# smellslikeml/distributed-deep-learning-workshop

Hardware: AMD Instinct MI355X
Metric: images/sec (whole node) ResNet-50 224px (higher is better)
Workload: dtype bf16; 1 GPU; model=resnet50, global_batch=256, per_gpu_batch=256, image_size=224, parallelism=dp1, hip_ops=True, conv_routes=hip

## Files before the change

ddlw_amd/ops/abi.py:

```python
from __future__ import annotations

import ctypes
from ctypes import POINTER, c_char_p, c_float, c_int, c_long, c_ulonglong


class Ptr(ctypes.c_void_p):

    @classmethod
    def from_param(cls, v):
        if v is None or isinstance(v, int):
            return ctypes.c_void_p(v)
        return ctypes.c_void_p(v.data_ptr())


def long_array(values):
    return (c_long * len(values))(*values)


def int_array(values):
    return (c_int * len(values))(*values)


_P, _I, _L, _F = Ptr, c_int, c_long, c_float

# ... 9 lines not shown
    "ddlw_bn_grad_finalize": (_I, [_P, _P, _P, _P, _I, _I, _P]),
    "ddlw_bn_bwd_dx": (_I, [_P] * 10 + [_L, _I, _I, _P]),
    "ddlw_maxpool3x3s2_fwd": (_I, [_P, _P, _P] + [_I] * 6 + [_P]),
    "ddlw_maxpool3x3s2_bwd": (_I, [_P, _P, _P] + [_I] * 6 + [_P]),
    "ddlw_gap_fwd": (_I, [_P, _P, _I, _I, _I, _P]),
    "ddlw_gap_bwd": (_I, [_P, _P, _I, _I, _I, _P]),
    "ddlw_softmax_ce": (_I, [_P, _P, _P, _P, _I, _I, _F, _P]),
    "ddlw_dropout_fwd": (_I, [_P, _P, _P, _L, _F, c_ulonglong, _P]),
    "ddlw_dropout_bwd": (_I, [_P, _P, _P, _L, _F, _P]),
    "ddlw_argmax_rows": (_I, [_P, _P, _L, _I, _P]),
    "ddlw_accuracy": (_I, [_P, _P, _P, _L, _I, _P]),
    "ddlw_normalize_u8": (_I, [_P, _P, _L, _P]),
    "ddlw_fused_sgd": (_I, [_P, _I, _L, _F, _F, _F, _I, _P]),
    "ddlw_fused_adam": (_I, [_P, _I, _L, _F, _F, _F, _F, _F, _F, _F, _P]),
    "ddlw_depthwise_fwd": (_I, [_P, _P, _P] + [_I] * 10 + [_P]),
    "ddlw_depthwise_fwd_ep": (_I, [_P] * 5 + [_I] * 9 + [_P]),
    "ddlw_depthwise_dgrad": (_I, [_P, _P, _P] + [_I] * 10 + [_P]),
    "ddlw_depthwise_wgrad_nparts": (_I, [_L, _I]),
    "ddlw_depthwise_wgrad": (_I, [_P, _P, _P, _P] + [_I] * 10 + [_P]),
    "ddlw_pw_conv_fwd": (_I, [_P] * 6 + [_I, _L, _I, _I, _P]),
    "ddlw_pw_conv_nparts": (_I, [_L, _I, _P]),
    "ddlw_pw_conv_fwd_stats": (_I, [_P] * 5 + [_L, _I, _I, _P]),
    "ddlw_conv_fwd_nparts": (_L, [_I] * 8),
    "ddlw_conv_fwd_igemm": (_I, [_P] * 13 + [_I] * 15 + [_P]),
    "ddlw_conv_dgrad_s2m": (_I, [_P] * 4 + [_I] * 9
                            + [POINTER(c_long), POINTER(c_long), POINTER(c_int), _P]),
    "ddlw_conv_wgrad": (_I, [_P] * 5 + [_I] * 12 + [_P]),
    "ddlw_stem_repack": (_I, [_P, _P, _I, _I, _I, _P]),
    "ddlw_conv_stem": (_I, [_P] * 4 + [_I] * 8 + [_P, _P, _I, _P]),
    "ddlw_stem_wgrad": (_I, [_P] * 5 + [_I] * 7 + [_P]),
}


def apply(cdll, on_missing) -> None:
    for name, (restype, argtypes) in SIGNATURES.items():
        try:
            fn = getattr(cdll, name)
        except AttributeError:
            on_missing(name)
            raise
        fn.restype = restype
        fn.argtypes = argtypes
```

ddlw_amd/ops/block.py:

```python
from __future__ import annotations

import os

import torch

from . import binding, conv_gemm


def fused_block_enabled() -> bool:
    return os.environ.get("DDLW_FUSED_BLOCK", "1") == "1"


def wgrad_stream_enabled() -> bool:
    return os.environ.get("DDLW_WGRAD_STREAM", "0") == "1"


_wgrad_streams = {}


def _wgrad_stream(device) -> "torch.cuda.Stream":
    s = _wgrad_streams.get(device)
    if s is None:
        s = _wgrad_streams[device] = torch.cuda.Stream(device=device)
    return s


def _cl(t: torch.Tensor) -> torch.Tensor:
    return t.contiguous(memory_format=torch.channels_last)


def _fwd_conv(x, w, stride, padding, hip_fwd):
    if hip_fwd:
        return conv_gemm.conv_fwd_kernel(x, w.to(torch.bfloat16), stride, padding)
    return torch.nn.functional.conv2d(x, w.to(x.dtype), None, stride, padding)


def _dgrad_bn_reduce(dy, conv_in, weight, stride, padding, hip_dgrad,
                     x_bn, mask, mean, rstd):
    st = stride[0] if isinstance(stride, (tuple, list)) else stride
    if (hip_dgrad and st == 1
            and os.environ.get("DDLW_FUSED_BNB", "1") == "1"):
        dx, parts, np_ = conv_gemm.conv_dgrad_kernel(
            dy, weight.to(torch.bfloat16), conv_in.shape, padding, stride,
            bnb=(x_bn, mask, mean, rstd))
        db, dg = binding.bn_grad_finalize_parts(
            parts[0], parts[1], np_, x_bn.shape[1])
        return dx, db, dg
# ... 2 lines not shown
    db, dg = binding.bn_bwd_reduce(dx, mask, x_bn, mean, rstd,
                                   mask is not None)
    return dx, db, dg


def _fwd_conv_bn_stats(x, w, stride, padding, hip_fwd, bn):
    if hip_fwd and os.environ.get("DDLW_FUSED_BN_STATS", "1") == "1":
        t, parts, np_ = conv_gemm.conv_fwd_kernel(
            x, w.to(torch.bfloat16), stride, padding, bn_parts=True)
        rows = t.shape[0] * t.shape[2] * t.shape[3]
        mean, rstd = binding.bn_finalize_parts(
            parts[0], parts[1], np_, rows, t.shape[1], bn.eps, bn.momentum,
            bn.running_mean, bn.running_var)
        return t, mean, rstd
    t = _fwd_conv(x, w, stride, padding, hip_fwd)
    mean, rstd = binding.bn_stats(t, bn.eps, bn.momentum,
                                  bn.running_mean, bn.running_var)
    return t, mean, rstd


class _BottleneckFn(torch.autograd.Function):

    @staticmethod
    def forward(ctx, x, w1, g1, b1, w2, g2, b2, w3, g3, b3, wd, gd, bd, block):
        bn1, bn2, bn3 = block.bn1, block.bn2, block.bn3
        stride = block.stride
        mode = os.environ.get("DDLW_CONV", "auto")
        x = _cl(x)

        if wd is not None:
            dsc = block.downsample.conv
            dsbn = block.downsample.bn
            conv_gemm.available(dsc, x, mode)
            rdf, rdd, rdg = getattr(dsc, "_ddlw_route", (False, False, False))
            td, md, sd = _fwd_conv_bn_stats(x, wd, stride, 0, rdf, dsbn)
            res, _ = binding.bn_apply(td, None, md, sd, gd, bd, False)
            dsbn.num_batches_tracked += 1
        else:
            rdd = rdg = False
            td = md = sd = None
            res = x

        conv_gemm.available(block.conv1, x, mode)
        r1f, r1d, r1g = getattr(block.conv1, "_ddlw_route", (False, False, False))
        t1, m1, s1 = _fwd_conv_bn_stats(x, w1, 1, 0, r1f, bn1)
        a1, mask1 = binding.bn_apply(t1, None, m1, s1, g1, b1, True)

        conv_gemm.available(block.conv2, a1, mode)
        r2f, r2d, r2g = getattr(block.conv2, "_ddlw_route", (False, False, False))
        t2, m2, s2 = _fwd_conv_bn_stats(a1, w2, stride, 1, r2f, bn2)
        a2, mask2 = binding.bn_apply(t2, None, m2, s2, g2, b2, True)

        conv_gemm.available(block.conv3, a2, mode)
        r3f, r3d, r3g = getattr(block.conv3, "_ddlw_route", (False, False, False))
        t3, m3, s3 = _fwd_conv_bn_stats(a2, w3, 1, 0, r3f, bn3)
        out, mask3 = binding.bn_apply(t3, res, m3, s3, g3, b3, True)

        for bn in (bn1, bn2, bn3):
            bn.num_batches_tracked += 1
        ctx.save_for_backward(x, w1, g1, w2, g2, w3, g3, wd, gd,
                              t1, a1, t2, a2, t3, td,
                              mask1, mask2, mask3,
                              m1, s1, m2, s2, m3, s3, md, sd)
        ctx.routes = ((r1d, r1g), (r2d, r2g), (r3d, r3g), (rdd, rdg))
        ctx.stride = stride
        return out

    @staticmethod
    def backward(ctx, dy):
        (x, w1, g1, w2, g2, w3, g3, wd, gd,
         t1, a1, t2, a2, t3, td,
         mask1, mask2, mask3,
         m1, s1, m2, s2, m3, s3, md, sd) = ctx.saved_tensors
        (r1d, r1g), (r2d, r2g), (r3d, r3g), (rdd, rdg) = ctx.routes
        stride = ctx.stride
        dy = _cl(dy)
        if dy.dtype != torch.bfloat16:
            dy = dy.to(torch.bfloat16)

        use_side = wgrad_stream_enabled() and dy.is_cuda
        main = torch.cuda.current_stream() if use_side else None
        side = _wgrad_stream(dy.device) if use_side else None
        side_evs = []

        def wgrad(dy_t, x_t, w, st, pd, hip_g):
            if not use_side:
                _, dw = conv_gemm.conv_backward(dy_t, x_t, w, st, pd,
                                                False, hip_g, need_dx=False)
                return dw
            ready = torch.cuda.Event()
            ready.record(main)
            side.wait_event(ready)
            with torch.cuda.stream(side):
                dy_t.record_stream(side)
                x_t.record_stream(side)
                _, dw = conv_gemm.conv_backward(dy_t, x_t, w, st, pd,
                                                False, hip_g, need_dx=False)
                done = torch.cuda.Event()
                done.record(side)
            side_evs.append((done, dw))
            return dw

        db3, dg3 = binding.bn_bwd_reduce(dy, mask3, t3, m3, s3, True)
        dt3, dres = binding.bn_bwd_dx(dy, mask3, t3, m3, s3, g3, db3, dg3,
                                      True, True)
        dw3 = wgrad(dt3, a2, w3, 1, 0, r3g)
        da2, db2, dg2 = _dgrad_bn_reduce(dt3, a2, w3, 1, 0, r3d,
                                         t2, mask2, m2, s2)
        dt2, _ = binding.bn_bwd_dx(da2, mask2, t2, m2, s2, g2, db2, dg2,
                                   True, False)
        dw2 = wgrad(dt2, a1, w2, stride, 1, r2g)
        da1, db1, dg1 = _dgrad_bn_reduce(dt2, a1, w2, stride, 1, r2d,
                                         t1, mask1, m1, s1)
        dt1, _ = binding.bn_bwd_dx(da1, mask1, t1, m1, s1, g1, db1, dg1,
                                   True, False)

        dwd = dgd = dbd = None
        if wd is not None:
            dbd, dgd = binding.bn_bwd_reduce(dres, None, td, md, sd, False)
            dtd, _ = binding.bn_bwd_dx(dres, None, td, md, sd, gd, dbd, dgd,
                                       False, False)
            dwd = wgrad(dtd, x, wd, stride, 0, rdg)
            dxd, _ = conv_gemm.conv_backward(dtd, x, wd, stride, 0, rdd, False,
                                             need_dw=False)
            join = dxd
        else:
            join = dres
        dw1 = wgrad(dt1, x, w1, 1, 0, r1g)
        dx, _ = conv_gemm.conv_backward(dt1, x, w1, 1, 0, r1d, False,
                                        need_dw=False, acc=join)

        for done, dw in side_evs:
            main.wait_event(done)
            dw.record_stream(main)

        return (dx, dw1, dg1, db1, dw2, dg2, db2, dw3, dg3, db3,
                dwd, dgd, dbd, None)


@torch.no_grad()
def bottleneck_eval_forward(block, x: torch.Tensor) -> torch.Tensor:
    x = _cl(x)
    stride = block.stride

    def _conv_ep(inp, w, bn, relu, acc=None, st=1, pad=0):
        return conv_gemm.conv_fwd_kernel(
            inp, w.to(torch.bfloat16), st, pad, acc=acc,
            ep=(*bn.folded_scale_bias(), relu))

    if block.downsample is not None:
        ds = block.downsample
        res = _conv_ep(x, ds.conv.weight, ds.bn, False, st=stride, pad=0)
    else:
        res = x
    a1 = _conv_ep(x, block.conv1.weight, block.bn1, True)
    a2 = _conv_ep(a1, block.conv2.weight, block.bn2, True, st=stride, pad=1)
    return _conv_ep(a2, block.conv3.weight, block.bn3, True, acc=res)


def bottleneck_eval_fusable(block, x: torch.Tensor) -> bool:
# ... 26 lines not shown
        return False
    if not (x.is_cuda and x.dtype == torch.bfloat16):
        return False
    if os.environ.get("DDLW_DISABLE_HIP_OPS", "0") == "1":
        return False
    bns = [block.bn1, block.bn2, block.bn3]
    if block.downsample is not None:
        bns.append(block.downsample.bn)
    for bn in bns:
        if bn.weight.dtype != torch.float32 or bn.running_mean.dtype != torch.float32:
            return False
        if not binding.supported_channels(bn.num_features):
            return False
    return True


def bottleneck_forward(block, x: torch.Tensor) -> torch.Tensor:
    if block.downsample is not None:
        wd = block.downsample.conv.weight
        gd = block.downsample.bn.weight
        bd = block.downsample.bn.bias
    else:
        wd = gd = bd = None
    return _BottleneckFn.apply(
        x,
        block.conv1.weight, block.bn1.weight, block.bn1.bias,
        block.conv2.weight, block.bn2.weight, block.bn2.bias,
        block.conv3.weight, block.bn3.weight, block.bn3.bias,
        wd, gd, bd,
        block,
    )
```

ddlw_amd/ops/conv_gemm.py:

```python
from __future__ import annotations

import json
import os
from pathlib import Path
from typing import Tuple

import torch

from .abi import int_array, long_array
from .runtime import launch, query

_DISPATCH_PATH = Path(__file__).resolve().parent / "conv_dispatch.json"
_dispatch = None


def _table() -> dict:
    global _dispatch
    if _dispatch is None:
        if _DISPATCH_PATH.exists():
            _dispatch = json.loads(_DISPATCH_PATH.read_text())
        else:
            _dispatch = {}
    return _dispatch

# ... 24 lines not shown
        t = torch.zeros(64, dtype=torch.bfloat16, device=device)
        _zpage[device] = t
    return t


def _route(kind: str, shape_key: str, mode: str, supported: bool) -> bool:
    if not supported:
        return False
    if mode == "hip":
        return True
    if mode == "stock":
        return False
    ent = _table().get(shape_key)
    if ent is None:
        return False
    return ent.get(kind, "stock") == "hip"


def _pair(v) -> Tuple[int, int]:
    return (v, v) if isinstance(v, int) else (int(v[0]), int(v[1]))


def _igemm(x, w, y, N, H, W, C, K, Ho, Wo, R, S, stride, pad, oH, oW, oS,
           acc=None, parts=None, bnb=(None,) * 4, ep=(None, None, 0)):
    ps, pq = (None, None) if parts is None else (parts[0], parts[1])
    launch("conv_fwd_igemm", x, w, y, _zero_page(x.device), acc, ps, pq, *bnb,
           ep[0], ep[1], 1 if ep[2] else 0,
           N, H, W, C, K, Ho, Wo, R, S, stride, pad, oH, oW, oS)


def conv_fwd_kernel(x: torch.Tensor, weight: torch.Tensor, stride, padding,
                    acc: torch.Tensor = None, bn_parts: bool = False,
                    bnb=None, ep=None):
    n, c, h, w = x.shape
    k, _, r, s = weight.shape
    st, _ = _pair(stride)
    pd, _ = _pair(padding)
    ho = (h + 2 * pd - r) // st + 1
    wo = (w + 2 * pd - s) // st + 1
    x = x.contiguous(memory_format=torch.channels_last)
    weight = weight.contiguous(memory_format=torch.channels_last)
    y = torch.empty((n, k, ho, wo), dtype=torch.bfloat16, device=x.device,
                    memory_format=torch.channels_last)
    if acc is not None:
        assert acc.shape == y.shape and acc.dtype == torch.bfloat16
        acc = acc.contiguous(memory_format=torch.channels_last)
    bnb_args, ep_args = (None,) * 4, (None, None, 0)
    parts = np_ = None
    if ep is not None:
        ep_args = ep
    elif bnb is not None or bn_parts:
        if bnb is not None:
            bx, bmask, bmean, brstd = bnb
            bx = bx.contiguous(memory_format=torch.channels_last)
            bnb_args = (bx, bmask, bmean, brstd)
        else:
            assert acc is None
        np_ = int(query("conv_fwd_nparts", n, c, k, ho, wo, r, s,
                        1 if bnb is not None else 0))
        parts = torch.empty(2, np_, k, dtype=torch.float32, device=x.device)
    _igemm(x, weight, y, n, h, w, c, k, ho, wo, r, s, st, pd, ho, wo, 1,
           acc, parts, bnb_args, ep_args)
    return y if parts is None else (y, parts, np_)


def wgrad_supported(C: int, K: int) -> bool:
    return C % 8 == 0 and K % 8 == 0


def _wgrad_split(M: int, K: int, C: int, RS: int) -> int:
    bk = 128 if K >= 128 else 64
    bc = 128 if C >= 128 else 64
    base = ((K + bk - 1) // bk) * ((C + bc - 1) // bc) * RS
    split = max(1, min(1024 // max(base, 1), 1024, M // 64 or 1))
    return split


def conv_wgrad_kernel(dy: torch.Tensor, x: torch.Tensor, weight_shape,
                      stride, padding) -> torch.Tensor:
    n, c, h, w = x.shape
    k, _, r, s = weight_shape
    st, _ = _pair(stride)
    pd, _ = _pair(padding)
    ho, wo = dy.shape[2], dy.shape[3]
    M = n * ho * wo
    split = _wgrad_split(M, k, c, r * s)
    x = x.contiguous(memory_format=torch.channels_last)
    dy = dy.contiguous(memory_format=torch.channels_last)
    elems = k * r * s * c
    slab = torch.empty(split * elems, dtype=torch.float32, device=x.device)
    dw = torch.empty((k, c, r, s), dtype=torch.bfloat16, device=x.device,
                     memory_format=torch.channels_last)
    launch("conv_wgrad", dy, x, _zero_page(x.device), slab, dw,
           n, h, w, c, k, ho, wo, r, s, st, pd, split)
    return dw


def conv_dgrad_kernel(dy: torch.Tensor, weight: torch.Tensor, in_shape,
                      padding, stride=1, acc: torch.Tensor = None, bnb=None):
    k, c, r, s = weight.shape
    pd, _ = _pair(padding)
    st, _ = _pair(stride)
    wt = weight.flip(2, 3).permute(1, 0, 2, 3)
    wt = wt.contiguous(memory_format=torch.channels_last)
    if st == 1:
        return conv_fwd_kernel(dy, wt, 1, r - 1 - pd, acc=acc, bnb=bnb)
    assert acc is None, "fused accumulate: stride-1 dgrad only"
    assert bnb is None, "fused BN-bwd reduce: stride-1 dgrad only"
    if st == 2 and r == 3 and pd == 1:
        return _conv_dgrad_s2_3x3(dy, weight, in_shape)
    assert st == 2 and r == 1 and pd == 0, "scatter dgrad: 1x1 s2 pad0 only"
    n, _, ho, wo = dy.shape
    _, _, ih, iw = in_shape
    dy = dy.contiguous(memory_format=torch.channels_last)
    dx = torch.empty((n, c, ih, iw), dtype=torch.bfloat16, device=dy.device,
                     memory_format=torch.channels_last).zero_()
    _igemm(dy, wt, dx, n, ho, wo, k, c, ho, wo, 1, 1, 1, 0, ih, iw, 2)
    return dx


def _raw_fwd_scatter(x, wflat, y_ptr, N, H, W, C, K, Ho, Wo, R, S,
                     oH, oW, oS):
    _igemm(x, wflat, y_ptr, N, H, W, C, K, Ho, Wo, R, S, 1, 0, oH, oW, oS)


def _conv_dgrad_s2_3x3(dy: torch.Tensor, weight: torch.Tensor, in_shape) -> torch.Tensor:
    k, c, _, _ = weight.shape
    n, _, ih, iw = in_shape
    ho, wo = dy.shape[2], dy.shape[3]
    dy = dy.contiguous(memory_format=torch.channels_last)
# ... 12 lines not shown
    if ih % 2 == 0 and iw % 2 == 0 and k % 64 == 0:
        wcat = torch.cat([wf.permute(0, 2, 3, 1).reshape(-1)
                          for *_, wf in classes])
        woffs = [0]
        for *_, wf in classes[:-1]:
            woffs.append(woffs[-1] + wf.numel())
        launch("conv_dgrad_s2m", dy, wcat, dx, _zero_page(dy.device),
               n, ho, wo, k, c, ih // 2, iw // 2, ih, iw,
               long_array(woffs),
               long_array([off for _, _, _, _, off, _ in classes]),
               int_array([v for _, _, nr, ns, _, _ in classes for v in (nr, ns)]))
        return dx
    for dh, dw_, nr, ns, off_elems, wf in classes:
        oh = (ih - dh + 1) // 2
        ow = (iw - dw_ + 1) // 2
        _raw_fwd_scatter(
            dy, wf, dx.data_ptr() + off_elems * dx.element_size(),
            n, ho, wo, k, c, oh, ow, nr, ns, ih, iw, 2,
        )
    return dx


def conv_backward(dy, x, weight, stride, padding, hip_dgrad, hip_wgrad,
                  need_dx=True, need_dw=True, acc=None):
    dy = dy.contiguous(memory_format=torch.channels_last)
    if dy.is_cuda and dy.dtype != torch.bfloat16:
        dy = dy.to(torch.bfloat16)
    st, _ = _pair(stride)
    dx = dw = None
    if need_dx and hip_dgrad:
        fuse = acc if st == 1 else None
        dx = conv_dgrad_kernel(dy, weight.to(torch.bfloat16), x.shape,
                               padding, stride, acc=fuse)
        if acc is not None and fuse is None:
            dx = dx + acc
    if need_dw and hip_wgrad:
        dw = conv_wgrad_kernel(dy, x, weight.shape, stride, padding)
        if dw.dtype != weight.dtype:
            dw = dw.to(weight.dtype)
    if (need_dw and dw is None) or (need_dx and dx is None):
        mask_dx = bool(need_dx and dx is None)
        mask_dw = bool(need_dw and dw is None)
        w16 = weight.to(dy.dtype)
        gi, gw, _ = torch.ops.aten.convolution_backward(
            dy, x, w16, None,
            list(stride) if isinstance(stride, (tuple, list)) else [stride] * 2,
            list(padding) if isinstance(padding, (tuple, list)) else [padding] * 2,
            [1, 1], False, [0, 0], 1,
            [mask_dx, mask_dw, False],
        )
        if mask_dx:
            dx = gi if acc is None else gi + acc
        if mask_dw:
            dw = gw.to(weight.dtype)
    return dx, dw

# ... 134 lines not shown
```

ddlw_amd/ops/hip/conv_gemm.hip:

```cpp
#include "igemm.h"
#include <cstdlib>
#include <type_traits>

typedef __attribute__((ext_vector_type(8))) __bf16 bf16x8_v;
typedef __attribute__((ext_vector_type(4))) float f32x4_v;
typedef __attribute__((ext_vector_type(16))) float f32x16_v;

template <int MF, int NF, int BM, int BN, int WM, int WN, typename ACC>
__device__ __forceinline__ void bn_partials_16(
    const ACC& acc, float* __restrict__ bn_ps, float* __restrict__ bn_pq,
    long tile_m, int tile_n, int wr, int wc, long M, int K) {
  const int lane = threadIdx.x & 63;
  const int d_col = lane & 15;
  const int d_row0 = (lane >> 4) * 4;
  float s[NF], q[NF];
  #pragma unroll
  for (int ni = 0; ni < NF; ++ni) { s[ni] = 0.f; q[ni] = 0.f; }
  #pragma unroll
  for (int mi = 0; mi < MF; ++mi)
    #pragma unroll
    for (int ni = 0; ni < NF; ++ni)
      #pragma unroll
      for (int qq = 0; qq < 4; ++qq) {
        long m = tile_m * BM + (long)wr * WM + mi * 16 + d_row0 + qq;
// ... 8 lines not shown
  for (int ni = 0; ni < NF; ++ni) {
    s[ni] += __shfl_xor(s[ni], 16, 64);
    s[ni] += __shfl_xor(s[ni], 32, 64);
    q[ni] += __shfl_xor(q[ni], 16, 64);
    q[ni] += __shfl_xor(q[ni], 32, 64);
  }
  if (lane < 16) {
    const long prow_ = tile_m * (BM / WM) + wr;
    #pragma unroll
    for (int ni = 0; ni < NF; ++ni) {
      int j = tile_n * BN + wc * WN + ni * 16 + d_col;
      if (j < K) {
        bn_ps[prow_ * K + j] = s[ni];
        bn_pq[prow_ * K + j] = q[ni];
      }
    }
  }
}

template <int MF, int NF, int BM, int BN, int WM, int WN, typename ACC,
          typename OutRow>
__device__ __forceinline__ void bnb_partials_16(
    const ACC& acc, const bf16_t* __restrict__ accp,
    const bf16_t* __restrict__ bx, const unsigned char* __restrict__ bmask,
    const float* __restrict__ bmean, const float* __restrict__ brstd,
    float* __restrict__ p_db, float* __restrict__ p_dg,
    long tile_m, int tile_n, int wr, int wc, long M, int K, OutRow out_row) {
  const int lane = threadIdx.x & 63;
  const int d_col = lane & 15;
  const int d_row0 = (lane >> 4) * 4;
  float s[NF], q[NF], mn[NF], rs[NF];
  #pragma unroll
  for (int ni = 0; ni < NF; ++ni) {
    int j = tile_n * BN + wc * WN + ni * 16 + d_col;
    s[ni] = 0.f;
    q[ni] = 0.f;
    mn[ni] = (j < K) ? bmean[j] : 0.f;
    rs[ni] = (j < K) ? brstd[j] : 0.f;
  }
  #pragma unroll
  for (int mi = 0; mi < MF; ++mi)
    #pragma unroll
    for (int ni = 0; ni < NF; ++ni) {
      int j = tile_n * BN + wc * WN + ni * 16 + d_col;
      if (j >= K) continue;
      #pragma unroll
      for (int qq = 0; qq < 4; ++qq) {
        long m = tile_m * BM + (long)wr * WM + mi * 16 + d_row0 + qq;
        if (m < M) {
          long oi = out_row(m) * K + j;
          float v = acc[mi][ni][qq];
          if (accp) {
            union { unsigned i; float f; } ca;
            ca.i = (unsigned)accp[oi] << 16;
            v += ca.f;
          }
          union { unsigned i; float f; } cv;
          cv.i = (unsigned)f2b(v) << 16;
          bool on = true;
          if (bmask)
            on = (bmask[oi >> 3] >> (j & 7)) & 1;
          if (on) {
            union { unsigned i; float f; } cx;
            cx.i = (unsigned)bx[oi] << 16;
            s[ni] += cv.f;
            q[ni] += cv.f * (cx.f - mn[ni]) * rs[ni];
          }
        }
      }
    }
  #pragma unroll
  for (int ni = 0; ni < NF; ++ni) {
    s[ni] += __shfl_xor(s[ni], 16, 64);
    s[ni] += __shfl_xor(s[ni], 32, 64);
    q[ni] += __shfl_xor(q[ni], 16, 64);
    q[ni] += __shfl_xor(q[ni], 32, 64);
  }
  if (lane < 16) {
    const long prow_ = tile_m * (BM / WM) + wr;
    #pragma unroll
    for (int ni = 0; ni < NF; ++ni) {
      int j = tile_n * BN + wc * WN + ni * 16 + d_col;
      if (j < K) {
        p_db[prow_ * K + j] = s[ni];
        p_dg[prow_ * K + j] = q[ni];
      }
    }
  }
}

struct S2Class {
  long woff;
  long yoff;
  int R, S;
};
struct S2Quad {
  S2Class c[4];
};

template <int BM, int BN, bool EPI_LDS, int BUFS, bool M32EN = true>
__global__ __launch_bounds__(256) void k_conv_fwd_igemm(
    const bf16_t* __restrict__ x, const bf16_t* __restrict__ w,
    bf16_t* __restrict__ y, const bf16_t* __restrict__ zpage,
    int N, int H, int W_, int C, int K, int Ho, int Wo,
    int R, int S, int stride, int pad, int nwg_swz,
    int oH, int oW, int oS,
    unsigned long long magic_wo, unsigned shift_wo,
    unsigned long long magic_ho, unsigned shift_ho,
    const bf16_t* __restrict__ accp,
    float* __restrict__ bn_ps,
    float* __restrict__ bn_pq,
    const bf16_t* __restrict__ bnb_x,
    const unsigned char* __restrict__ bnb_mask,
    const float* __restrict__ bnb_mean,
    const float* __restrict__ bnb_rstd,
    const float* __restrict__ ep_scale = nullptr,
    const float* __restrict__ ep_bias = nullptr,
    int ep_relu = 0,
    int s2_merged = 0, S2Quad quad = {}) {
  if (s2_merged) {
    const S2Class& cc = quad.c[blockIdx.y];
    w += cc.woff;
    y += cc.yoff;
    R = cc.R;
    S = cc.S;
  }
  constexpr int BK = 64;
  constexpr int WM = BM / 2, WN = BN / 2;
  constexpr int MF = WM / 16, NF = WN / 16;
  constexpr int AP = BM / 32;
  constexpr int BP = BN / 32;
  constexpr int BUF = (BM + BN) * BK;
// ... 225 lines not shown
      }
    } else {
      float eps_[NF], epb_[NF];
      if (ep_scale) {
        #pragma unroll
        for (int ni = 0; ni < NF; ++ni) {
          int j = tile_n * BN + wc * WN + ni * 16 + d_col;
          eps_[ni] = (j < K) ? ep_scale[j] : 0.f;
          epb_[ni] = (j < K) ? ep_bias[j] : 0.f;
        }
      }
      #pragma unroll
      for (int mi = 0; mi < MF; ++mi) {
        #pragma unroll
        for (int ni = 0; ni < NF; ++ni) {
          int j = tile_n * BN + wc * WN + ni * 16 + d_col;
          if (j >= K) continue;
          #pragma unroll
          for (int q = 0; q < 4; ++q) {
            long m = tile_m * BM + wr * WM + mi * 16 + d_row0 + q;
            if (m < M) {
              long oi = out_row(m) * K + j;
              float v = acc[mi][ni][q];
              if (ep_scale) v = v * eps_[ni] + epb_[ni];
              if (accp) v += b2f(accp[oi]);
              if (ep_relu) v = fmaxf(v, 0.f);
              y[oi] = f2b(v);
            }
          }
        }
      }
      if (bn_ps) {
        if (bnb_x)
          bnb_partials_16<MF, NF, BM, BN, WM, WN>(
              acc, accp, bnb_x, bnb_mask, bnb_mean, bnb_rstd, bn_ps, bn_pq,
              tile_m, tile_n, wr, wc, M, K, out_row);
        else
          bn_partials_16<MF, NF, BM, BN, WM, WN>(acc, bn_ps, bn_pq, tile_m,
                                                 tile_n, wr, wc, M, K);
      }
    }
    return;
  }
  constexpr int WNP = WN + 8;
  bf16_t* lC = smem + wave * (WM * WNP);
  if constexpr (M32) {
    #pragma unroll
    for (int mi = 0; mi < MF2; ++mi)
      #pragma unroll
      for (int ni = 0; ni < NF2; ++ni)
        #pragma unroll
        for (int reg = 0; reg < 16; ++reg) {
          int row = (reg & 3) + 8 * (reg >> 2) + d_rbase32;
          lC[(mi * 32 + row) * WNP + ni * 32 + d_col32] =
              f2b(acc2[mi][ni][reg]);
        }
  } else {
    #pragma unroll
    for (int mi = 0; mi < MF; ++mi)
      #pragma unroll
      for (int ni = 0; ni < NF; ++ni)
        #pragma unroll
        for (int q = 0; q < 4; ++q)
          lC[(mi * 16 + d_row0 + q) * WNP + ni * 16 + d_col] =
              f2b(acc[mi][ni][q]);
  }
  constexpr int CPL = WN / 8;
  constexpr int RPI = 64 / CPL;
  const int e_row = lane / CPL;
  const int e_ch = lane % CPL;
  const long m_base = tile_m * BM + wr * WM;
  const int j_base = tile_n * BN + wc * WN + e_ch * 8;
  float eps8[8], epb8[8];
  if (ep_scale) {
    #pragma unroll
    for (int e = 0; e < 8; ++e) {
      int j = j_base + e;
      eps8[e] = (j < K) ? ep_scale[j] : 0.f;
      epb8[e] = (j < K) ? ep_bias[j] : 0.f;
    }
// ... 2 lines not shown
    float f = b2f(v) * eps8[e] + epb8[e] + accv;
    if (ep_relu) f = fmaxf(f, 0.f);
    return f2b(f);
  };
  float s8[8], q8[8], bnm8[8], bnr8[8];
  #pragma unroll
  for (int e = 0; e < 8; ++e) { s8[e] = 0.f; q8[e] = 0.f; }
  if (bn_ps && bnb_x) {
    #pragma unroll
    for (int e = 0; e < 8; ++e) {
      int j = j_base + e;
      bnm8[e] = (j < K) ? bnb_mean[j] : 0.f;
      bnr8[e] = (j < K) ? bnb_rstd[j] : 0.f;
    }
  }
  #pragma unroll
  for (int it = 0; it < WM / RPI; ++it) {
    const int row = it * RPI + e_row;
    const long m = m_base + row;
    uint4 val = *reinterpret_cast<const uint4*>(lC + row * WNP + e_ch * 8);
    if (m < M) {
      const long orow = out_row(m);
      if (j_base + 8 <= K) {
        if (ep_scale) {
          uint4 a{0, 0, 0, 0};
          if (accp)
            a = *reinterpret_cast<const uint4*>(accp + orow * K + j_base);
          uint4 o;
          unsigned* ow = &o.x;
          const unsigned* vw = &val.x;
          const unsigned* aw = &a.x;
          #pragma unroll
          for (int d = 0; d < 4; ++d) {
            float alo = accp ? b2f((bf16_t)(aw[d] & 0xffff)) : 0.f;
            float ahi = accp ? b2f((bf16_t)(aw[d] >> 16)) : 0.f;
            bf16_t lo = ep_apply((bf16_t)(vw[d] & 0xffff), 2 * d, alo);
            bf16_t hi = ep_apply((bf16_t)(vw[d] >> 16), 2 * d + 1, ahi);
            ow[d] = (unsigned)lo | ((unsigned)hi << 16);
          }
          *reinterpret_cast<uint4*>(y + orow * K + j_base) = o;
        } else if (accp) {
          uint4 a = *reinterpret_cast<const uint4*>(accp + orow * K + j_base);
          auto addpair = [&](unsigned v, unsigned aw) -> unsigned {
            bf16_t lo = f2b(b2f((bf16_t)(v & 0xffff)) + b2f((bf16_t)(aw & 0xffff)));
            bf16_t hi = f2b(b2f((bf16_t)(v >> 16)) + b2f((bf16_t)(aw >> 16)));
            return (unsigned)lo | ((unsigned)hi << 16);
          };
          val.x = addpair(val.x, a.x);
          val.y = addpair(val.y, a.y);
          val.z = addpair(val.z, a.z);
          val.w = addpair(val.w, a.w);
          *reinterpret_cast<uint4*>(y + orow * K + j_base) = val;
        } else {
          *reinterpret_cast<uint4*>(y + orow * K + j_base) = val;
        }
        if (bn_ps) {
          if (bnb_x) {
            unsigned mb = bnb_mask ? bnb_mask[(orow * K + j_base) >> 3] : 0xffu;
            uint4 xv = *reinterpret_cast<const uint4*>(bnb_x + orow * K + j_base);
            #pragma unroll
            for (int e = 0; e < 8; ++e) {
              unsigned wd = (e < 2) ? val.x : (e < 4) ? val.y : (e < 6) ? val.z : val.w;
              unsigned xw = (e < 2) ? xv.x : (e < 4) ? xv.y : (e < 6) ? xv.z : xv.w;
              if ((mb >> e) & 1) {
                float f = b2f((bf16_t)(wd >> ((e & 1) * 16)));
                float xf = b2f((bf16_t)(xw >> ((e & 1) * 16)));
                s8[e] += f;
                q8[e] += f * (xf - bnm8[e]) * bnr8[e];
              }
            }
          } else {
            #pragma unroll
            for (int e = 0; e < 8; ++e) {
              unsigned wd = (e < 2) ? val.x : (e < 4) ? val.y : (e < 6) ? val.z : val.w;
              float f = b2f((bf16_t)(wd >> ((e & 1) * 16)));
              s8[e] += f;
              q8[e] += f * f;
            }
          }
        }
      } else {
        #pragma unroll
        for (int e = 0; e < 8; ++e) {
          if (j_base + e < K) {
            unsigned wd = (e < 2) ? val.x : (e < 4) ? val.y : (e < 6) ? val.z : val.w;
            bf16_t ov = (bf16_t)(wd >> ((e & 1) * 16));
            if (ep_scale) {
              float av = accp ? b2f(accp[orow * K + j_base + e]) : 0.f;
              ov = ep_apply(ov, e, av);
            } else if (accp)
              ov = f2b(b2f(ov) + b2f(accp[orow * K + j_base + e]));
            y[orow * K + j_base + e] = ov;
            if (bn_ps) {
              float f = b2f(ov);
              if (bnb_x) {
                bool on = !bnb_mask ||
                          ((bnb_mask[(orow * K + j_base) >> 3] >> e) & 1);
                if (on) {
                  s8[e] += f;
                  q8[e] += f * (b2f(bnb_x[orow * K + j_base + e]) - bnm8[e]) *
                           bnr8[e];
                }
              } else {
                s8[e] += f;
                q8[e] += f * f;
              }
            }
          }
        }
      }
    }
  }
  if (bn_ps) {
    #pragma unroll
// ... 231 lines not shown
            long oi = out_row(m) * K + j;
            float v = acc[mi][ni][q];
            if constexpr (decltype(has_acc)::value) v += b2f(accp[oi]);
            y[oi] = f2b(v);
          }
        }
      }
    }
  };
  if (accp)
    epilogue(std::true_type{});
  else
    epilogue(std::false_type{});
  (void)bn_ps; (void)bn_pq; (void)bnb_x; (void)bnb_mask;
  (void)bnb_mean; (void)bnb_rstd;
}

struct TilePick {
  int bm, bn, bufs, wvm;
  bool epi_lds, wide, m32;
};

static TilePick pick_tile(long M, int K, int C, int T, bool want_stats,
                          bool want_bnb = false, bool want_ep = false) {
  int mfma_pref, wide_pref;
  {
    const char* e = getenv("DDLW_CONV_MFMA");
    mfma_pref = (e && e[0] == '3') ? 32 : 16;
    const char* e2 = getenv("DDLW_CONV_WIDE");
    wide_pref = e2 ? (e2[0] == '0' ? 0 : 1) : -1;
  }
  TilePick p{};
  p.m32 = (mfma_pref == 32) && !want_stats && !want_bnb;
  const bool wide_auto = false;
  if (!want_bnb && !want_stats && !want_ep &&
      ((wide_pref == 1 && K >= 128 && T >= 4) || (wide_pref == -1 && wide_auto))) {
    p.wide = true;
    p.bm = 256;
    p.bn = (K >= 256) ? 256 : 128;
    p.bufs = (p.bn == 256) ? 2 : 3;
    p.wvm = 4;
    return p;
  }
  p.bm = 128;
  p.wvm = 2;
  p.bn = (K >= 128) ? 128 : (K >= 64 ? 64 : 32);
  p.epi_lds = (T <= 4) || want_bnb;
  p.bufs = (T == 1) ? 1 : 2;
  return p;
}

DDLW_EXPORT long ddlw_conv_fwd_nparts(int N, int C, int K, int Ho, int Wo,
                                      int R, int S, int bnb) {
  long M = (long)N * Ho * Wo;
  const int T = R * S * (C / 64);
  TilePick p = pick_tile(M, K, C, T, true, bnb != 0);
  return cdiv(M, p.bm) * p.wvm;
}

DDLW_EXPORT int ddlw_conv_fwd_igemm(const void* x, const void* w, void* y,
                                    const void* zpage, const void* acc,
                                    void* bn_ps, void* bn_pq,
                                    const void* bnb_x, const void* bnb_mask,
                                    const void* bnb_mean, const void* bnb_rstd,
                                    const void* ep_scale, const void* ep_bias,
                                    int ep_relu,
                                    int N, int H, int W_, int C, int K,
                                    int Ho, int Wo, int R, int S, int stride,
                                    int pad, int oH, int oW, int oS,
                                    void* stream) {
  if (C % 64 != 0) {
    ddlw_set_error("conv_fwd_igemm: C must be a multiple of 64");
    return 2;
  }
  long M = (long)N * Ho * Wo;
  if (M >= (1ll << 31)) {
    ddlw_set_error("conv_fwd_igemm: M >= 2^31 unsupported");
    return 2;
  }
  unsigned long long mg_wo, mg_ho;
  unsigned sh_wo, sh_ho;
  make_magic((unsigned)Wo, &mg_wo, &sh_wo);
  make_magic((unsigned)Ho, &mg_ho, &sh_ho);
  const int T = R * S * (C / 64);
  hipStream_t st = (hipStream_t)stream;
  const bool want_stats = bn_ps != nullptr;
  const bool want_bnb = bnb_x != nullptr;
  const bool want_ep = ep_scale != nullptr;
  TilePick p = pick_tile(M, K, C, T, want_stats, want_bnb, want_ep);
  if (p.wide) {
    long grid = cdiv(M, 256) * cdiv(K, p.bn);
#define WIDE_LAUNCH(BN_, NB_)                                                  \
    hipLaunchKernelGGL((k_conv_igemm_wide<256, BN_, NB_>), dim3((int)grid),    \
                       dim3(512), 0, st, (const bf16_t*)x, (const bf16_t*)w,   \
                       (bf16_t*)y, (const bf16_t*)zpage, N, H, W_, C, K, Ho,   \
                       Wo, R, S, stride, pad, (int)grid, oH, oW, oS, mg_wo,    \
                       sh_wo, mg_ho, sh_ho, (const bf16_t*)acc,                \
                       (float*)bn_ps, (float*)bn_pq, (const bf16_t*)bnb_x,     \
                       (const unsigned char*)bnb_mask,                         \
                       (const float*)bnb_mean, (const float*)bnb_rstd)
    if (p.bn == 256)
      WIDE_LAUNCH(256, 2);
    else
      WIDE_LAUNCH(128, 3);
#undef WIDE_LAUNCH
    DDLW_CHECK_LAUNCH();
  }
  with_int<128, 64, 32>(p.bn, [&](auto BN) {
    with_bool(p.epi_lds, [&](auto EPI) {
      with_int<1, 2>(p.bufs, [&](auto BUFS) {
        with_bool(p.m32, [&](auto M32) {
          long grid = cdiv(M, 128) * cdiv(K, decltype(BN)::value);
          hipLaunchKernelGGL(
              (k_conv_fwd_igemm<128, decltype(BN)::value, decltype(EPI)::value,
                                decltype(BUFS)::value, decltype(M32)::value>),
              dim3((int)grid), dim3(256), 0, st, (const bf16_t*)x,
              (const bf16_t*)w, (bf16_t*)y, (const bf16_t*)zpage, N, H, W_, C,
              K, Ho, Wo, R, S, stride, pad, (int)grid, oH, oW, oS, mg_wo,
              sh_wo, mg_ho, sh_ho, (const bf16_t*)acc, (float*)bn_ps,
              (float*)bn_pq, (const bf16_t*)bnb_x,
              (const unsigned char*)bnb_mask, (const float*)bnb_mean,
              (const float*)bnb_rstd, (const float*)ep_scale,
              (const float*)ep_bias, ep_relu);
        });
      });
    });
  });
  DDLW_CHECK_LAUNCH();
}

DDLW_EXPORT int ddlw_conv_dgrad_s2m(const void* dy, const void* wcat, void* dx,
                                    const void* zpage, int N, int Ho, int Wo,
                                    int Kdy, int Cdx, int oh, int ow, int ih,
                                    int iw, const long* woffs,
                                    const long* yoffs, const int* crs,
                                    void* stream) {
  if (Kdy % 64 != 0) {
    ddlw_set_error("conv_dgrad_s2m: dy channels must be a multiple of 64");
    return 2;
  }
  long M = (long)N * oh * ow;
  if (M >= (1ll << 31)) {
// ... 3 lines not shown
  unsigned long long mg_wo, mg_ho;
  unsigned sh_wo, sh_ho;
  make_magic((unsigned)ow, &mg_wo, &sh_wo);
  make_magic((unsigned)oh, &mg_ho, &sh_ho);
  S2Quad q;
  for (int i = 0; i < 4; ++i)
    q.c[i] = S2Class{woffs[i], yoffs[i], crs[2 * i], crs[2 * i + 1]};
  hipStream_t st = (hipStream_t)stream;
  int s2epi = 1;
  {
    const char* e = getenv("DDLW_S2_EPI");
    if (e && e[0] == '0') s2epi = 0;
  }
  with_bool(Cdx >= 128, [&](auto WIDE_N) {
    with_bool(s2epi != 0, [&](auto EPI) {
      constexpr int BN = decltype(WIDE_N)::value ? 128 : 64;
      long gx = cdiv(M, 128) * cdiv(Cdx, BN);
      hipLaunchKernelGGL(
          (k_conv_fwd_igemm<128, BN, decltype(EPI)::value, 2, false>),
          dim3((int)gx, 4), dim3(256), 0, st, (const bf16_t*)dy,
          (const bf16_t*)wcat, (bf16_t*)dx, (const bf16_t*)zpage, N, Ho, Wo,
          Kdy, Cdx, oh, ow, 2, 2, 1, 0, (int)gx, ih, iw, 2, mg_wo, sh_wo,
          mg_ho, sh_ho, nullptr, nullptr, nullptr, nullptr, nullptr, nullptr,
          nullptr, nullptr, nullptr, 0, 1, q);
    });
  });
  DDLW_CHECK_LAUNCH();
}
```

Baseline: 8752 images/sec.

## Fuse residual ReLU-mask join and next block's BN3 backward reduce into conv1 dgrad

The bottleneck backward pass no longer materializes the masked residual gradient `dres`. The conv1 dgrad epilogue instead adds `dy` with the BN3 ReLU bitmask applied, and the downsample BN backward reads `dy` and the mask directly. A per-block link object passes the upstream block's BN3 forward tensors into this block's conv1 dgrad. The dgrad kernel then also emits BN3 reduce partials, so the upstream block skips its own `bn_bwd_reduce` pass over `dy`. This removes several full-activation read and write passes per block, at the cost of new kernel template variants, more bookkeeping state checked by tensor version, and masked epilogue loads.

```diff
diff --git a/ddlw_amd/ops/abi.py b/ddlw_amd/ops/abi.py
--- a/ddlw_amd/ops/abi.py
+++ b/ddlw_amd/ops/abi.py
@@ -55,7 +55,7 @@
     "ddlw_pw_conv_nparts": (_I, [_L, _I, _P]),
     "ddlw_pw_conv_fwd_stats": (_I, [_P] * 5 + [_L, _I, _I, _P]),
     "ddlw_conv_fwd_nparts": (_L, [_I] * 8),
-    "ddlw_conv_fwd_igemm": (_I, [_P] * 13 + [_I] * 15 + [_P]),
+    "ddlw_conv_fwd_igemm": (_I, [_P] * 14 + [_I] * 15 + [_P]),
     "ddlw_conv_dgrad_s2m": (_I, [_P] * 4 + [_I] * 9
                             + [POINTER(c_long), POINTER(c_long), POINTER(c_int), _P]),
     "ddlw_conv_wgrad": (_I, [_P] * 5 + [_I] * 12 + [_P]),
diff --git a/ddlw_amd/ops/block.py b/ddlw_amd/ops/block.py
--- a/ddlw_amd/ops/block.py
+++ b/ddlw_amd/ops/block.py
@@ -23,6 +23,47 @@
     if s is None:
         s = _wgrad_streams[device] = torch.cuda.Stream(device=device)
     return s
+
+
+def fused_join_enabled() -> bool:
+    return os.environ.get("DDLW_FUSED_JOIN", "1") != "0"
+
+
+def fused_bn3_enabled() -> bool:
+    return os.environ.get("DDLW_FUSED_BN3", "1") != "0"
+
+
+class _Bn3Link:
+
+    FIELDS = ("t3", "mask3", "m3", "s3", "parts", "nparts", "dx",
+              "dx_version")
+    __slots__ = FIELDS + ("__weakref__",)
+
+    def __init__(self):
+        self.clear()
+
+    def clear(self):
+        self.t3 = self.mask3 = self.m3 = self.s3 = None
+        self.parts = self.nparts = self.dx = self.dx_version = None
+
+    def armed(self) -> bool:
+        return self.t3 is not None
+
+    def take_bnb(self):
+        bnb = (self.t3, self.mask3, self.m3, self.s3)
+        self.t3 = self.mask3 = self.m3 = self.s3 = None
+        return bnb
+
+    def put(self, parts, nparts, dx):
+        self.parts, self.nparts, self.dx = parts, nparts, dx
+        self.dx_version = dx._version
+
+    def matches(self, dy: torch.Tensor) -> bool:
+        dx = self.dx
+        return (dx is not None and dy.data_ptr() == dx.data_ptr()
+                and dy.shape == dx.shape and dy.dtype == dx.dtype
+                and dy.stride() == dx.stride()
+                and dy._version == self.dx_version)
 
 
 def _cl(t: torch.Tensor) -> torch.Tensor:
@@ -71,7 +112,8 @@
 class _BottleneckFn(torch.autograd.Function):
 
     @staticmethod
-    def forward(ctx, x, w1, g1, b1, w2, g2, b2, w3, g3, b3, wd, gd, bd, block):
+    def forward(ctx, x, w1, g1, b1, w2, g2, b2, w3, g3, b3, wd, gd, bd, block,
+                link_in=None, link_out=None):
         bn1, bn2, bn3 = block.bn1, block.bn2, block.bn3
         stride = block.stride
         mode = os.environ.get("DDLW_CONV", "auto")
@@ -113,6 +155,11 @@
                               m1, s1, m2, s2, m3, s3, md, sd)
         ctx.routes = ((r1d, r1g), (r2d, r2g), (r3d, r3g), (rdd, rdg))
         ctx.stride = stride
+        ctx.link_in = link_in
+        ctx.link_out = link_out
+        if link_out is not None:
+            link_out.t3, link_out.mask3 = t3, mask3
+            link_out.m3, link_out.s3 = m3, s3
         return out
 
     @staticmethod
@@ -123,6 +170,12 @@
          m1, s1, m2, s2, m3, s3, md, sd) = ctx.saved_tensors
         (r1d, r1g), (r2d, r2g), (r3d, r3g), (rdd, rdg) = ctx.routes
         stride = ctx.stride
+        link_in, link_out = ctx.link_in, ctx.link_out
+        parts3 = None
+        if link_out is not None:
+            if link_out.matches(dy) and fused_bn3_enabled():
+                parts3 = (link_out.parts, link_out.nparts)
+            link_out.clear()
         dy = _cl(dy)
         if dy.dtype != torch.bfloat16:
             dy = dy.to(torch.bfloat16)
@@ -150,9 +203,19 @@
             side_evs.append((done, dw))
             return dw
 
-        db3, dg3 = binding.bn_bwd_reduce(dy, mask3, t3, m3, s3, True)
+        if not fused_join_enabled():
+            join_fused = False
+        elif wd is not None:
+            join_fused = True
+        else:
+            join_fused = bool(r1d)
+        if parts3 is not None:
+            db3, dg3 = binding.bn_grad_finalize_parts(
+                parts3[0][0], parts3[0][1], parts3[1], t3.shape[1])
+        else:
+            db3, dg3 = binding.bn_bwd_reduce(dy, mask3, t3, m3, s3, True)
         dt3, dres = binding.bn_bwd_dx(dy, mask3, t3, m3, s3, g3, db3, dg3,
-                                      True, True)
+                                      True, not join_fused)
         dw3 = wgrad(dt3, a2, w3, 1, 0, r3g)
         da2, db2, dg2 = _dgrad_bn_reduce(dt3, a2, w3, 1, 0, r3d,
                                          t2, mask2, m2, s2)
@@ -166,25 +229,40 @@
 
         dwd = dgd = dbd = None
         if wd is not None:
-            dbd, dgd = binding.bn_bwd_reduce(dres, None, td, md, sd, False)
-            dtd, _ = binding.bn_bwd_dx(dres, None, td, md, sd, gd, dbd, dgd,
-                                       False, False)
+            if join_fused:
+                dbd, dgd = binding.bn_bwd_reduce(dy, mask3, td, md, sd, True)
+                dtd, _ = binding.bn_bwd_dx(dy, mask3, td, md, sd, gd, dbd,
+                                           dgd, True, False)
+            else:
+                dbd, dgd = binding.bn_bwd_reduce(dres, None, td, md, sd, False)
+                dtd, _ = binding.bn_bwd_dx(dres, None, td, md, sd, gd, dbd,
+                                           dgd, False, False)
             dwd = wgrad(dtd, x, wd, stride, 0, rdg)
             dxd, _ = conv_gemm.conv_backward(dtd, x, wd, stride, 0, rdd, False,
                                              need_dw=False)
-            join = dxd
-        else:
-            join = dres
+            join, join_mask = dxd, None
+        elif join_fused:
+            join, join_mask = dy, mask3
+        else:
+            join, join_mask = dres, None
         dw1 = wgrad(dt1, x, w1, 1, 0, r1g)
-        dx, _ = conv_gemm.conv_backward(dt1, x, w1, 1, 0, r1d, False,
-                                        need_dw=False, acc=join)
+        if (link_in is not None and link_in.armed() and r1d
+                and fused_bn3_enabled()):
+            dx, parts, np_ = conv_gemm.conv_dgrad_kernel(
+                dt1, w1.to(torch.bfloat16), x.shape, 0, 1, acc=join,
+                acc_mask=join_mask, bnb=link_in.take_bnb())
+            link_in.put(parts, np_, dx)
+        else:
+            dx, _ = conv_gemm.conv_backward(dt1, x, w1, 1, 0, r1d, False,
+                                            need_dw=False, acc=join,
+                                            acc_mask=join_mask)
 
         for done, dw in side_evs:
             main.wait_event(done)
             dw.record_stream(main)
 
         return (dx, dw1, dg1, db1, dw2, dg2, db2, dw3, dg3, db3,
-                dwd, dgd, dbd, None)
+                dwd, dgd, dbd, None, None, None)
 
 
 @torch.no_grad()
@@ -257,11 +335,15 @@
         bd = block.downsample.bn.bias
     else:
         wd = gd = bd = None
-    return _BottleneckFn.apply(
+    link_in = getattr(x, "_ddlw_bn3_link", None)
+    link_out = _Bn3Link()
+    out = _BottleneckFn.apply(
         x,
         block.conv1.weight, block.bn1.weight, block.bn1.bias,
         block.conv2.weight, block.bn2.weight, block.bn2.bias,
         block.conv3.weight, block.bn3.weight, block.bn3.bias,
         wd, gd, bd,
-        block,
+        block, link_in, link_out,
     )
+    out._ddlw_bn3_link = link_out
+    return out
diff --git a/ddlw_amd/ops/conv_gemm.py b/ddlw_amd/ops/conv_gemm.py
--- a/ddlw_amd/ops/conv_gemm.py
+++ b/ddlw_amd/ops/conv_gemm.py
@@ -70,16 +70,18 @@
 
 
 def _igemm(x, w, y, N, H, W, C, K, Ho, Wo, R, S, stride, pad, oH, oW, oS,
-           acc=None, parts=None, bnb=(None,) * 4, ep=(None, None, 0)):
+           acc=None, parts=None, bnb=(None,) * 4, ep=(None, None, 0),
+           acc_mask=None):
     ps, pq = (None, None) if parts is None else (parts[0], parts[1])
-    launch("conv_fwd_igemm", x, w, y, _zero_page(x.device), acc, ps, pq, *bnb,
+    launch("conv_fwd_igemm", x, w, y, _zero_page(x.device), acc, acc_mask,
+           ps, pq, *bnb,
            ep[0], ep[1], 1 if ep[2] else 0,
            N, H, W, C, K, Ho, Wo, R, S, stride, pad, oH, oW, oS)
 
 
 def conv_fwd_kernel(x: torch.Tensor, weight: torch.Tensor, stride, padding,
                     acc: torch.Tensor = None, bn_parts: bool = False,
-                    bnb=None, ep=None):
+                    bnb=None, ep=None, acc_mask: torch.Tensor = None):
     n, c, h, w = x.shape
     k, _, r, s = weight.shape
     st, _ = _pair(stride)
@@ -93,6 +95,9 @@
     if acc is not None:
         assert acc.shape == y.shape and acc.dtype == torch.bfloat16
         acc = acc.contiguous(memory_format=torch.channels_last)
+    if acc_mask is not None and acc is not None:
+        assert (acc_mask.dtype == torch.uint8 and acc_mask.is_contiguous()
+                and acc_mask.numel() * 8 == y.numel())
     bnb_args, ep_args = (None,) * 4, (None, None, 0)
     parts = np_ = None
     if ep is not None:
@@ -108,7 +113,7 @@
                         1 if bnb is not None else 0))
         parts = torch.empty(2, np_, k, dtype=torch.float32, device=x.device)
     _igemm(x, weight, y, n, h, w, c, k, ho, wo, r, s, st, pd, ho, wo, 1,
-           acc, parts, bnb_args, ep_args)
+           acc, parts, bnb_args, ep_args, acc_mask)
     return y if parts is None else (y, parts, np_)
 
 
@@ -145,15 +150,18 @@
 
 
 def conv_dgrad_kernel(dy: torch.Tensor, weight: torch.Tensor, in_shape,
-                      padding, stride=1, acc: torch.Tensor = None, bnb=None):
+                      padding, stride=1, acc: torch.Tensor = None, bnb=None,
+                      acc_mask: torch.Tensor = None):
     k, c, r, s = weight.shape
     pd, _ = _pair(padding)
     st, _ = _pair(stride)
     wt = weight.flip(2, 3).permute(1, 0, 2, 3)
     wt = wt.contiguous(memory_format=torch.channels_last)
     if st == 1:
-        return conv_fwd_kernel(dy, wt, 1, r - 1 - pd, acc=acc, bnb=bnb)
-    assert acc is None, "fused accumulate: stride-1 dgrad only"
+        return conv_fwd_kernel(dy, wt, 1, r - 1 - pd, acc=acc, bnb=bnb,
+                               acc_mask=acc_mask)
+    assert acc is None and acc_mask is None, \
+        "fused accumulate: stride-1 dgrad only"
     assert bnb is None, "fused BN-bwd reduce: stride-1 dgrad only"
     if st == 2 and r == 3 and pd == 1:
         return _conv_dgrad_s2_3x3(dy, weight, in_shape)
@@ -212,7 +220,10 @@
 
 
 def conv_backward(dy, x, weight, stride, padding, hip_dgrad, hip_wgrad,
-                  need_dx=True, need_dw=True, acc=None):
+                  need_dx=True, need_dw=True, acc=None, acc_mask=None):
+    if acc_mask is not None and not (need_dx and hip_dgrad
+                                     and _pair(stride)[0] == 1):
+        raise ValueError("conv_backward: acc_mask needs the stride-1 HIP dgrad")
     dy = dy.contiguous(memory_format=torch.channels_last)
     if dy.is_cuda and dy.dtype != torch.bfloat16:
         dy = dy.to(torch.bfloat16)
@@ -221,7 +232,7 @@
     if need_dx and hip_dgrad:
         fuse = acc if st == 1 else None
         dx = conv_dgrad_kernel(dy, weight.to(torch.bfloat16), x.shape,
-                               padding, stride, acc=fuse)
+                               padding, stride, acc=fuse, acc_mask=acc_mask)
         if acc is not None and fuse is None:
             dx = dx + acc
     if need_dw and hip_wgrad:
diff --git a/ddlw_amd/ops/hip/conv_gemm.hip b/ddlw_amd/ops/hip/conv_gemm.hip
--- a/ddlw_amd/ops/hip/conv_gemm.hip
+++ b/ddlw_amd/ops/hip/conv_gemm.hip
@@ -54,6 +54,7 @@
           typename OutRow>
 __device__ __forceinline__ void bnb_partials_16(
     const ACC& acc, const bf16_t* __restrict__ accp,
+    const unsigned char* __restrict__ accmask,
     const bf16_t* __restrict__ bx, const unsigned char* __restrict__ bmask,
     const float* __restrict__ bmean, const float* __restrict__ brstd,
     float* __restrict__ p_db, float* __restrict__ p_dg,
@@ -85,6 +86,7 @@
           if (accp) {
             union { unsigned i; float f; } ca;
             ca.i = (unsigned)accp[oi] << 16;
+            if (accmask && !((accmask[oi >> 3] >> (j & 7)) & 1)) ca.f = 0.f;
             v += ca.f;
           }
           union { unsigned i; float f; } cv;
@@ -130,7 +132,8 @@
   S2Class c[4];
 };
 
-template <int BM, int BN, bool EPI_LDS, int BUFS, bool M32EN = true>
+template <int BM, int BN, bool EPI_LDS, int BUFS, bool M32EN = true,
+          bool ACC_EARLY = false, bool MASKED = false>
 __global__ __launch_bounds__(256) void k_conv_fwd_igemm(
     const bf16_t* __restrict__ x, const bf16_t* __restrict__ w,
     bf16_t* __restrict__ y, const bf16_t* __restrict__ zpage,
@@ -140,6 +143,7 @@
     unsigned long long magic_wo, unsigned shift_wo,
     unsigned long long magic_ho, unsigned shift_ho,
     const bf16_t* __restrict__ accp,
+    const unsigned char* __restrict__ acc_mask,
     float* __restrict__ bn_ps,
     float* __restrict__ bn_pq,
     const bf16_t* __restrict__ bnb_x,
@@ -411,9 +415,15 @@
             if (m < M) {
               long oi = out_row(m) * K + j;
               float v = acc[mi][ni][q];
-              if (ep_scale) v = v * eps_[ni] + epb_[ni];
-              if (accp) v += b2f(accp[oi]);
-              if (ep_relu) v = fmaxf(v, 0.f);
+              if constexpr (MASKED) {
+                float a = b2f(accp[oi]);
+                if (!((acc_mask[oi >> 3] >> (j & 7)) & 1)) a = 0.f;
+                v += a;
+              } else {
+                if (ep_scale) v = v * eps_[ni] + epb_[ni];
+                if (accp) v += b2f(accp[oi]);
+                if (ep_relu) v = fmaxf(v, 0.f);
+              }
               y[oi] = f2b(v);
             }
           }
@@ -422,8 +432,8 @@
       if (bn_ps) {
         if (bnb_x)
           bnb_partials_16<MF, NF, BM, BN, WM, WN>(
-              acc, accp, bnb_x, bnb_mask, bnb_mean, bnb_rstd, bn_ps, bn_pq,
-              tile_m, tile_n, wr, wc, M, K, out_row);
+              acc, accp, MASKED ? acc_mask : nullptr, bnb_x, bnb_mask, bnb_mean, bnb_rstd, bn_ps,
+              bn_pq, tile_m, tile_n, wr, wc, M, K, out_row);
         else
           bn_partials_16<MF, NF, BM, BN, WM, WN>(acc, bn_ps, bn_pq, tile_m,
                                                  tile_n, wr, wc, M, K);
@@ -433,6 +443,7 @@
   }
   constexpr int WNP = WN + 8;
   bf16_t* lC = smem + wave * (WM * WNP);
+  constexpr bool acc_early = ACC_EARLY && !M32;
   if constexpr (M32) {
     #pragma unroll
     for (int mi = 0; mi < MF2; ++mi)
@@ -445,6 +456,28 @@
               f2b(acc2[mi][ni][reg]);
         }
   } else {
+    if constexpr (acc_early) {
+        #pragma unroll
+        for (int mi = 0; mi < MF; ++mi) {
+          #pragma unroll
+          for (int ni = 0; ni < NF; ++ni) {
+            int j = tile_n * BN + wc * WN + ni * 16 + d_col;
+            if (j >= K) continue;
+            #pragma unroll
+            for (int q = 0; q < 4; ++q) {
+              long m = tile_m * BM + wr * WM + mi * 16 + d_row0 + q;
+              if (m < M) {
+                long oi = out_row(m) * K + j;
+                float a = b2f(accp[oi]);
+                if constexpr (MASKED) {
+                  if (!((acc_mask[oi >> 3] >> (j & 7)) & 1)) a = 0.f;
+                }
+                acc[mi][ni][q] += a;
+              }
+            }
+          }
+        }
+    }
     #pragma unroll
     for (int mi = 0; mi < MF; ++mi)
       #pragma unroll
@@ -493,7 +526,7 @@
     if (m < M) {
       const long orow = out_row(m);
       if (j_base + 8 <= K) {
-        if (ep_scale) {
+        if (!MASKED && ep_scale) {
           uint4 a{0, 0, 0, 0};
           if (accp)
             a = *reinterpret_cast<const uint4*>(accp + orow * K + j_base);
@@ -510,9 +543,20 @@
             ow[d] = (unsigned)lo | ((unsigned)hi << 16);
           }
           *reinterpret_cast<uint4*>(y + orow * K + j_base) = o;
-        } else if (accp) {
+        } else if (accp && !acc_early) {
           uint4 a = *reinterpret_cast<const uint4*>(accp + orow * K + j_base);
-          auto addpair = [&](unsigned v, unsigned aw) -> unsigned {
+          if constexpr (MASKED) {
+            const unsigned mb = acc_mask[(orow * K + j_base) >> 3];
+            auto keep = [&](int e) -> unsigned {
+              return (((mb >> e) & 1) ? 0xffffu : 0u) |
+                     (((mb >> (e + 1)) & 1) ? 0xffff0000u : 0u);
+            };
+            a.x &= keep(0);
+            a.y &= keep(2);
+            a.z &= keep(4);
+            a.w &= keep(6);
+          }
+          auto addpair =[&](unsigned v, unsigned aw) -> unsigned {
             bf16_t lo = f2b(b2f((bf16_t)(v & 0xffff)) + b2f((bf16_t)(aw & 0xffff)));
             bf16_t hi = f2b(b2f((bf16_t)(v >> 16)) + b2f((bf16_t)(aw >> 16)));
             return (unsigned)lo | ((unsigned)hi << 16);
@@ -556,11 +600,16 @@
           if (j_base + e < K) {
             unsigned wd = (e < 2) ? val.x : (e < 4) ? val.y : (e < 6) ? val.z : val.w;
             bf16_t ov = (bf16_t)(wd >> ((e & 1) * 16));
-            if (ep_scale) {
+            if (!MASKED && ep_scale) {
               float av = accp ? b2f(accp[orow * K + j_base + e]) : 0.f;
               ov = ep_apply(ov, e, av);
-            } else if (accp)
-              ov = f2b(b2f(ov) + b2f(accp[orow * K + j_base + e]));
+            } else if (accp && !acc_early) {
+              float av = b2f(accp[orow * K + j_base + e]);
+              if constexpr (MASKED) {
+                if (!((acc_mask[(orow * K + j_base) >> 3] >> e) & 1)) av = 0.f;
+              }
+              ov = f2b(b2f(ov) + av);
+            }
             y[orow * K + j_base + e] = ov;
             if (bn_ps) {
               float f = b2f(ov);
@@ -838,7 +887,8 @@
 };
 
 static TilePick pick_tile(long M, int K, int C, int T, bool want_stats,
-                          bool want_bnb = false, bool want_ep = false) {
+                          bool want_bnb = false, bool want_ep = false,
+                          bool want_mask = false) {
   int mfma_pref, wide_pref;
   {
     const char* e = getenv("DDLW_CONV_MFMA");
@@ -847,9 +897,9 @@
     wide_pref = e2 ? (e2[0] == '0' ? 0 : 1) : -1;
   }
   TilePick p{};
-  p.m32 = (mfma_pref == 32) && !want_stats && !want_bnb;
+  p.m32 = (mfma_pref == 32) && !want_stats && !want_bnb && !want_mask;
   const bool wide_auto = false;
-  if (!want_bnb && !want_stats && !want_ep &&
+  if (!want_bnb && !want_stats && !want_ep && !want_mask &&
       ((wide_pref == 1 && K >= 128 && T >= 4) || (wide_pref == -1 && wide_auto))) {
     p.wide = true;
     p.bm = 256;
@@ -876,6 +926,7 @@
 
 DDLW_EXPORT int ddlw_conv_fwd_igemm(const void* x, const void* w, void* y,
                                     const void* zpage, const void* acc,
+                                    const void* acc_mask,
                                     void* bn_ps, void* bn_pq,
                                     const void* bnb_x, const void* bnb_mask,
                                     const void* bnb_mean, const void* bnb_rstd,
@@ -889,6 +940,9 @@
     ddlw_set_error("conv_fwd_igemm: C must be a multiple of 64");
     return 2;
   }
+  if (acc_mask && (!acc || ep_scale || K % 8 != 0))
+    return ddlw_fail("conv_fwd_igemm",
+                     "acc_mask needs acc, no ep_scale and K a multiple of 8");
   long M = (long)N * Ho * Wo;
   if (M >= (1ll << 31)) {
     ddlw_set_error("conv_fwd_igemm: M >= 2^31 unsupported");
@@ -903,7 +957,8 @@
   const bool want_stats = bn_ps != nullptr;
   const bool want_bnb = bnb_x != nullptr;
   const bool want_ep = ep_scale != nullptr;
-  TilePick p = pick_tile(M, K, C, T, want_stats, want_bnb, want_ep);
+  TilePick p = pick_tile(M, K, C, T, want_stats, want_bnb, want_ep,
+                         acc_mask != nullptr);
   if (p.wide) {
     long grid = cdiv(M, 256) * cdiv(K, p.bn);
 #define WIDE_LAUNCH(BN_, NB_)                                                  \
@@ -922,6 +977,45 @@
 #undef WIDE_LAUNCH
     DDLW_CHECK_LAUNCH();
   }
+  if (acc && want_bnb && T > 4) {
+    with_int<128, 64, 32>(p.bn, [&](auto BN) {
+     with_bool(acc_mask != nullptr, [&](auto MSK) {
+      long grid = cdiv(M, 128) * cdiv(K, decltype(BN)::value);
+      hipLaunchKernelGGL(
+          (k_conv_fwd_igemm<128, decltype(BN)::value, true, 2, false, true,
+                            decltype(MSK)::value>),
+          dim3((int)grid), dim3(256), 0, st, (const bf16_t*)x,
+          (const bf16_t*)w, (bf16_t*)y, (const bf16_t*)zpage, N, H, W_, C, K,
+          Ho, Wo, R, S, stride, pad, (int)grid, oH, oW, oS, mg_wo, sh_wo,
+          mg_ho, sh_ho, (const bf16_t*)acc, (const unsigned char*)acc_mask,
+          (float*)bn_ps, (float*)bn_pq, (const bf16_t*)bnb_x,
+          (const unsigned char*)bnb_mask, (const float*)bnb_mean,
+          (const float*)bnb_rstd, nullptr, nullptr, 0);
+     });
+    });
+    DDLW_CHECK_LAUNCH();
+  }
+  if (acc_mask) {
+    with_int<128, 64, 32>(p.bn, [&](auto BN) {
+      with_bool(p.epi_lds, [&](auto EPI) {
+        with_int<1, 2>(p.bufs, [&](auto BUFS) {
+          long grid = cdiv(M, 128) * cdiv(K, decltype(BN)::value);
+          hipLaunchKernelGGL(
+              (k_conv_fwd_igemm<128, decltype(BN)::value, decltype(EPI)::value,
+                                decltype(BUFS)::value, false, false, true>),
+              dim3((int)grid), dim3(256), 0, st, (const bf16_t*)x,
+              (const bf16_t*)w, (bf16_t*)y, (const bf16_t*)zpage, N, H, W_, C,
+              K, Ho, Wo, R, S, stride, pad, (int)grid, oH, oW, oS, mg_wo,
+              sh_wo, mg_ho, sh_ho, (const bf16_t*)acc,
+              (const unsigned char*)acc_mask, (float*)bn_ps, (float*)bn_pq,
+              (const bf16_t*)bnb_x, (const unsigned char*)bnb_mask,
+              (const float*)bnb_mean, (const float*)bnb_rstd, nullptr, nullptr,
+              0);
+        });
+      });
+    });
+    DDLW_CHECK_LAUNCH();
+  }
   with_int<128, 64, 32>(p.bn, [&](auto BN) {
     with_bool(p.epi_lds, [&](auto EPI) {
       with_int<1, 2>(p.bufs, [&](auto BUFS) {
@@ -933,7 +1027,8 @@
               dim3((int)grid), dim3(256), 0, st, (const bf16_t*)x,
               (const bf16_t*)w, (bf16_t*)y, (const bf16_t*)zpage, N, H, W_, C,
               K, Ho, Wo, R, S, stride, pad, (int)grid, oH, oW, oS, mg_wo,
-              sh_wo, mg_ho, sh_ho, (const bf16_t*)acc, (float*)bn_ps,
+              sh_wo, mg_ho, sh_ho, (const bf16_t*)acc,
+              (const unsigned char*)acc_mask, (float*)bn_ps,
               (float*)bn_pq, (const bf16_t*)bnb_x,
               (const unsigned char*)bnb_mask, (const float*)bnb_mean,
               (const float*)bnb_rstd, (const float*)ep_scale,
@@ -983,7 +1078,7 @@
           (const bf16_t*)wcat, (bf16_t*)dx, (const bf16_t*)zpage, N, Ho, Wo,
           Kdy, Cdx, oh, ow, 2, 2, 1, 0, (int)gx, ih, iw, 2, mg_wo, sh_wo,
           mg_ho, sh_ho, nullptr, nullptr, nullptr, nullptr, nullptr, nullptr,
-          nullptr, nullptr, nullptr, 0, 1, q);
+          nullptr, nullptr, nullptr, nullptr, 0, 1, q);
     });
   });
   DDLW_CHECK_LAUNCH();
```

New measurement: 8898 images/sec, median of 6. 1.02x the previous value.
